# HanzhiC/TexPose

Hardware: AMD Instinct MI355X
Metric: rendered rays/sec (480x640x128 samples) + train iters/sec (higher is better)
Workload: dtype f32 carried as 2xf16 (f16x3 products, f32 accumulate); 1 GPU; Duck-like synthetic scene 480x640, 128 samples/ray, batch=1 image per GPU, forward render (render_by_slices mode='val', all pixels), per-sample outputs materialised; samples_per_ray=128, mlp_precision=f16x3, parallelism=images sharded across 1 GPU(s), no collective

## Files before the change

### texpose_amd/csrc/gen_wide_asm.py

```python
#!/usr/bin/env python3
import os
import sys

NCH = 115
EXPERIMENT = os.environ.get("TP_ASM_EXPERIMENT", "")
SPLIT = os.environ.get("TP_ASM_SPLIT", "mix")

VB = 160
def F_hi(slot): return VB + 8 * slot
def F_lo(slot): return VB + 8 * slot + 4
XB = [VB + 32, VB + 48]
T = VB + 64
VR = VB + 68
HACC = VB + 72
CLOBBER_V = list(range(XB[0], VR + 3))
BA, BB = 92, 94
CLOBBER_S = [BA, BA + 1, BB, BB + 1]
SET = {"P": 0, "Q": 128}


def vr(lo, n=4):
    return "v[%d:%d]" % (lo, lo + n - 1)


def ar(set_base, tile):
    lo = set_base + 16 * tile
    return "a[%d:%d]" % (lo, lo + 15)


def mfma(dst, a, b, c=None):
    return "v_mfma_f32_32x32x16_f16 %s, %s, %s, %s" % (dst, a, b, dst if c is None else c)


def conv(src_base, tile, g, bank):
    xh = XB[bank] + (g >> 2) * 4 + (g & 3)
    xl = XB[bank] + 8 + (g >> 2) * 4 + (g & 3)
    t0, t1, h0, h1 = T, T + 1, T + 2, T + 3
    a = src_base + 16 * tile + 2 * g
    head = ["v_accvgpr_read_b32 v%d, a%d" % (t0, a),
            "v_accvgpr_read_b32 v%d, a%d" % (t1, a + 1),
            "v_mul_f32 v%d, %%[kinv], v%d" % (t0, t0),
            "v_mul_f32 v%d, %%[kinv], v%d" % (t1, t1),
            "v_max_f32 v%d, 0, v%d" % (t0, t0),
            "v_max_f32 v%d, 0, v%d" % (t1, t1)]
    return head + split_ops(t0, t1, h0, h1, xh, xl) + ["v_pk_max_f16 %%[amax], %%[amax], v%d" % xh]


def split_ops(t0, t1, h0, h1, xh, xl):
    if SPLIT == "and":
        return ["v_and_b32 v%d, %%[mask], v%d" % (h0, t0),
                "v_and_b32 v%d, %%[mask], v%d" % (h1, t1),
                "v_sub_f32 v%d, v%d, v%d" % (t0, t0, h0),
                "v_sub_f32 v%d, v%d, v%d" % (t1, t1, h1),
                "v_cvt_pkrtz_f16_f32 v%d, v%d, v%d" % (xh, h0, h1),
                "v_cvt_pkrtz_f16_f32 v%d, v%d, v%d" % (xl, t0, t1)]
    return ["v_cvt_pkrtz_f16_f32 v%d, v%d, v%d" % (xh, t0, t1),
            "v_fma_mix_f32 v%d, -v%d, 1.0, v%d op_sel_hi:[1,0,0]" % (h0, xh, t0),
            "v_fma_mix_f32 v%d, -v%d, 1.0, v%d op_sel:[1,0,0] op_sel_hi:[1,0,0]" % (h1, xh, t1),
            "v_cvt_pkrtz_f16_f32 v%d, v%d, v%d" % (xl, h0, h1)]


MK = VB + 71
RB = 96


def rec_wr_off(r):
    return (r >> 2) * 4096 + (r & 3) * 128


def conv_rec(src_base, tile, g, bank, mask=True):
    c = conv(src_base, tile, g, bank)
    t0, t1 = T, T + 1
    r0, r1 = 2 * g, 2 * g + 1
    out = c[0:6]
    if EXPERIMENT != "recnolds":
        out += ["ds_write_b32 %%[recw], v%d offset:%d" % (t0, rec_wr_off(r0)),
                "ds_write_b32 %%[recw], v%d offset:%d" % (t1, rec_wr_off(r1))]
    else:
        out += ["s_nop 0", "s_nop 0"]
    if mask:
        out += ["v_cmp_lt_f32_e32 vcc, 0, v%d" % t0,
                "v_addc_co_u32_e32 v%d, vcc, v%d, v%d, vcc" % (MK, MK, MK),
                "v_cmp_lt_f32_e32 vcc, 0, v%d" % t1,
                "v_addc_co_u32_e32 v%d, vcc, v%d, v%d, vcc" % (MK, MK, MK)]
    out += c[6:]
    return out


def tile_regs(set_base, tile, k):
    lo = set_base + 16 * tile + 4 * k
    return "a[%d:%d]" % (lo, lo + 3)


def rec_reads(set_base, tile):
    if EXPERIMENT == "recnolds":
        return []
    return ["ds_read_b128 %s, %%[recr] offset:%d" % (tile_regs(set_base, tile, k), k * 4096) for k in range(4)]


def rec_store(set_base, tile, k):
    if EXPERIMENT in ("recnostore", "recnolds"):
        return "s_nop 0"
    policy = {"recplain": "", "recsc1": " sc1", "recsc01": " sc0 sc1"}.get(EXPERIMENT, " nt")
    return "global_store_dwordx4 %%[ro%d], %s, s[%d:%d] offset:%d%s" % (k & 1, tile_regs(set_base, tile, k), RB, RB + 1, (k >> 1) * 2048, policy)


def rec_advance():
    return ["s_add_u32 s%d, s%d, 0x1000" % (RB, RB), "s_addc_u32 s%d, s%d, 0" % (RB + 1, RB + 1)]


def rec_mask_store(w4):
    if EXPERIMENT in ("recnostore", "recnolds"):
        return []
    return ["v_bfrev_b32_e32 v%d, v%d" % (MK, MK),
            "global_store_dword %%[mkoff], v%d, %%[rbase] offset:%d" % (MK, w4 * 256)]


def split_even(instrs, n):
    k, out, pos = len(instrs), [], 0
    for i in range(n):
        take = (k - pos + (n - i) - 1) // (n - i)
        out.append(instrs[pos:pos + take])
        pos += take
    return out


def ring_prologue(e):
    e("s_waitcnt lgkmcnt(0)")
    e("s_nop 7")
    e("s_nop 7")
    e("s_lshl_b32 %[r0], %[buf], 15")
    for k, r in ((1, "r1"), (2, "r2")):
        e("s_add_i32 %%[t0], %%[buf], %d" % k)
        e("s_cmp_ge_i32 %[t0], 3")
        e("s_cselect_b32 %%[%s], 3, 0" % r)
        e("s_sub_i32 %%[t0], %%[t0], %%[%s]" % r)
        e("s_lshl_b32 %%[%s], %%[t0], 15" % r)
    for i, r in enumerate(("r0", "r1", "r2")):
        e("v_add_u32 v%d, %%[%s], %%[lane16]" % (VR + i, r))
        e("s_add_i32 %%[m%da], %%[ldswave], %%[%s]" % (i, r))
    e("s_add_i32 %[dch], %[chunk], 2")
    e("s_cmp_ge_i32 %[dch], %[nch]")
# ... 1 lines not shown
    e("s_sub_i32 %[dch], %[dch], %[t0]")


def dma_base():
    return ["s_lshl_b32 %[t0], %[dch], 15",
            "s_add_u32 s%d, %%[stream_lo], %%[t0]" % BA,
            "s_addc_u32 s%d, %%[stream_hi], 0" % (BA + 1),
            "s_add_u32 s%d, s%d, 0x1000" % (BB, BA),
            "s_addc_u32 s%d, s%d, 0" % (BB + 1, BA + 1)]


def dma_piece(e, k, dma_slot):
    if k == 0:
        e("s_mov_b32 m0, %%[m%da]" % dma_slot)
        e("s_nop 0")
    elif k == 4:
        e("s_add_i32 m0, %%[m%da], 0x1000" % dma_slot)
        e("s_nop 0")
    base = "s[%d:%d]" % ((BA, BA + 1) if k < 4 else (BB, BB + 1))
    if EXPERIMENT != "nodma":
        e("global_load_lds_dwordx4 %%[laneoff], %s offset:%d" % (base, (k & 3) * 1024))


def ring_epilogue(e, n_chunks):
    e("s_waitcnt lgkmcnt(0)")
    e("s_add_i32 %%[chunk], %%[chunk], %d" % n_chunks)
    e("s_cmp_ge_i32 %[chunk], %[nch]")
    e("s_cselect_b32 %[t0], %[nch], 0")
    e("s_sub_i32 %[chunk], %[chunk], %[t0]")
    e("s_add_i32 %%[buf], %%[buf], %d" % (n_chunks % 3))
    e("s_cmp_ge_i32 %[buf], 3")
    e("s_cselect_b32 %[t0], 3, 0")
    e("s_sub_i32 %[buf], %[buf], %[t0]")


def refill(e, slot, pair, npairs, cur, nxt):
    addr, off = (VR + cur, pair * 2048) if pair < npairs else (VR + nxt, (pair - npairs) * 2048)
    e("ds_read_b128 %s, v%d offset:%d" % (vr(F_hi(slot)), addr, off))
    e("ds_read_b128 %s, v%d offset:%d" % (vr(F_lo(slot)), addr, off + 1024))


def publish(e, young):
    e("s_waitcnt vmcnt(%d) lgkmcnt(0)" % (0 if EXPERIMENT == "nodma" else young))
    if EXPERIMENT != "nobarrier":
        e("s_barrier")


def chunk_groups(e, npairs, ts, mf, fill, free_after, pieces_per_group, tail=None, head=None, young_extra=0):
    ngroups = npairs // 2
    cur, nxt, dma = ts % 3, (ts + 1) % 3, (ts + 2) % 3
    pub_group = (npairs - 4) // 2
    for g in range(ngroups):
        q = 2 * g
        sa, sb = q % 4, (q + 1) % 4
        lines = mf(g)
        gaps = fill(g)
        e("s_waitcnt lgkmcnt(4)")
        for i in range(6):
            e(lines[i])
            if i == 0:
                for k in range(pieces_per_group):
                    dma_piece(e, g * pieces_per_group + k, dma)
                if head is not None:
                    for ins in head(g):
                        e(ins)
            if i < 5:
                for ins in gaps[i]:
                    e(ins)
            if i + 1 == free_after[0]:
                if g == pub_group:
                    publish(e, (g + 1) * pieces_per_group + (0 if EXPERIMENT in ("recnostore", "recnolds") else young_extra))
                refill(e, sa, q + 4, npairs, cur, nxt)
            if i + 1 == free_after[1]:
                refill(e, sb, q + 5, npairs, cur, nxt)
        if tail is not None:
            for ins in tail(g):
                e(ins)


def advance_dch():
    return ["s_add_i32 %[dch], %[dch], 1", "s_cmp_eq_u32 %[dch], %[nch]", "s_cselect_b32 %[dch], 0, %[dch]"]


def gen_wide(src, dst, rec=None):
    L = []
    e = L.append
    ring_prologue(e)
    cvf = (lambda *a: conv_rec(*a, mask=(rec == "mask"))) if rec else conv
    if rec:
        e("s_mov_b64 s[%d:%d], %%[rbase]" % (RB, RB + 1))
    for g in range(8):
        for ins in cvf(src, 0, g, 0):
            e(ins)
    if rec:
        for ins in rec_reads(src, 0):
            e(ins)
    for ins in dma_base():
        e(ins)
    for ts in range(8):
        bank = ts & 1

        def mf(g, bank=bank):
            s, t = g >> 2, (2 * g) & 7
            sa, sb = (2 * g) % 4, (2 * g + 1) % 4
            xh, xl = vr(XB[bank] + s * 4), vr(XB[bank] + 8 + s * 4)
            d0, d1 = ar(dst, t), ar(dst, t + 1)
            return [mfma(d0, vr(F_hi(sa)), xh), mfma(d1, vr(F_hi(sb)), xh), mfma(d0, vr(F_hi(sa)), xl),
                    mfma(d1, vr(F_hi(sb)), xl), mfma(d0, vr(F_lo(sa)), xh), mfma(d1, vr(F_lo(sb)), xh)]

        def fill(g, ts=ts, bank=bank):
            if rec:
                first, mid1, mid2, mid3, last = [], [], [], [], []
                if 1 <= g <= 4:
                    first = [rec_store(src, ts, g - 1)]
                if g == 5:
                    first = rec_advance()
                if g == 7 and ts < 7:
                    rd = rec_reads(src, ts + 1)
                    mid2, mid3 = mid2 + rd[0:2], mid3 + rd[2:4]
                    if rec == "mask" and not (ts & 1):
                        last = last + rec_mask_store(ts >> 1)
                if ts == 7:
                    return [first, mid1, mid2, mid3, last]
                cv = conv_rec(src, ts + 1, g, bank ^ 1, mask=(rec == "mask"))
                if rec == "mask":
                    return [first + cv[0:4], mid1 + cv[4:9], cv[9:14] + mid2, cv[14:18] + mid3, cv[18:19] + last]
                return [first + cv[0:4], mid1 + cv[4:8], cv[8:12] + mid2, cv[12:15] + mid3, last]
            if ts == 7:
                return [[], [], [], [], []]
            cv = conv(src, ts + 1, g, bank ^ 1)
            if EXPERIMENT == "noconv":
                return [[], [], [], [], []]
            return [[], cv[0:4], cv[4:8], cv[8:12], cv[12:13]]

        def tail(g, ts=ts):
            out = []
            if ts < 7:
                if 1 <= g <= 3:
                    out.append(advance_dch()[g - 1])
                if g == 7:
                    out += dma_base()
            return out

        def head(g, ts=ts):
            if g != (6 if rec else 0):
                return []
            return ["ds_read_b128 a[%d:%d], %%[nbias] offset:%d" % (src + 16 * ts + 4 * k, src + 16 * ts + 4 * k + 3, ts * 64 + k * 16)
                    for k in range(4)]

        extra = 0
        if rec:
            extra = 4 + (1 if (ts & 1) and rec == "mask" else 0)
        chunk_groups(e, 16, ts, mf, fill, (5, 6), 1, tail, head, young_extra=extra)
    ring_epilogue(e, 8)
    return L


def gen_extra(dst, ks):
    L = []
    e = L.append
    ring_prologue(e)
    for s in range(ks):
        e("ds_read_b128 %s, %%[stage] offset:%d" % (vr(XB[0] + s * 4), s * 8192))
        e("ds_read_b128 %s, %%[stage] offset:%d" % (vr(XB[0] + 8 + s * 4), s * 8192 + 4096))
    for ins in dma_base():
        e(ins)
    e("s_waitcnt lgkmcnt(0)")

    def mf(g):
        s, t = g >> 2, (2 * g) & 7
        sa, sb = (2 * g) % 4, (2 * g + 1) % 4
        xh, xl = vr(XB[0] + s * 4), vr(XB[0] + 8 + s * 4)
        d0, d1 = ar(dst, t), ar(dst, t + 1)
        return [mfma(d0, vr(F_hi(sa)), xh), mfma(d1, vr(F_hi(sb)), xh), mfma(d0, vr(F_hi(sa)), xl),
                mfma(d1, vr(F_hi(sb)), xl), mfma(d0, vr(F_lo(sa)), xh), mfma(d1, vr(F_lo(sb)), xh)]

    chunk_groups(e, 8 * ks, 0, mf, lambda g: [[], [], [], [], []], (5, 6), 2 // ks)
    ring_epilogue(e, 1)
    return L


def gen_head(src, rec=False):
    L = []
    e = L.append
    ring_prologue(e)
    if rec:
        e("s_mov_b64 s[%d:%d], %%[rbase]" % (RB, RB + 1))
    for g in range(8):
        for ins in (conv_rec(src, 0, g, 0) if rec else conv(src, 0, g, 0)):
            e(ins)
    def hold_reads(t):
        return rec_reads(src, t)

    if rec:
        for ins in hold_reads(0):
            e(ins)
    for ins in dma_base():
        e(ins)
    acc = vr(HACC, 16)

    def mf(g):
        bank = g & 1
        sa, sb = (2 * g) % 4, (2 * g + 1) % 4
        xh0, xh1 = vr(XB[bank]), vr(XB[bank] + 4)
        xl0, xl1 = vr(XB[bank] + 8), vr(XB[bank] + 12)
        first = mfma(acc, vr(F_hi(sa)), xh0, "0") if g == 0 else mfma(acc, vr(F_hi(sa)), xh0)
        return [first, mfma(acc, vr(F_hi(sa)), xl0), mfma(acc, vr(F_lo(sa)), xh0),
                mfma(acc, vr(F_hi(sb)), xh1), mfma(acc, vr(F_hi(sb)), xl1), mfma(acc, vr(F_lo(sb)), xh1)]

    def fill(g):
        cv = []
        if g < 7:
# ... 295 lines not shown
            vm += 1
        if q == n - 8:
            publish(e, vm)
            lg.drained()
        p = q + 8
        addr, off = (VR + cur, p * 1024) if p < n else (VR + nxt, (p - n) * 1024)
        lg.lds(e, "ds_read_b128 %s, v%d offset:%d" % (vr(F16(q % 8)), addr, off), slot=q % 8)
        for ins, is_lds in fill(q):
            if is_lds:
                lg.lds(e, ins)
            else:
                e(ins)
    for ins in (tail or []):
        e(ins)


def gen_wide16(src, dst):
    L = []
    e = L.append
    lg = Lgkm()
    ring_prologue(e)
    for ins in conv16_tile(src, 0, XB[0]):
        e(ins)
    for ins in dma_base():
        e(ins)
    for c in range(4):
        b = c & 1
        cv1 = split_even(conv16_tile(src, 2 * c + 1, XB[b] + 8), 15)
        cv2 = split_even(conv16_tile(src, 2 * c + 2, XB[b ^ 1]), 15) if c < 3 else [[] for _ in range(15)]

        def seed(tile, k):
            return ("ds_read_b128 a[%d:%d], %%[nbias] offset:%d" % (src + 16 * tile + 4 * k, src + 16 * tile + 4 * k + 3,
                                                                   tile * 64 + k * 16), True)

        def fill(q, c=c, cv1=cv1, cv2=cv2):
            out = []
            if 1 <= q <= 4:
                out.append(seed(2 * c, q - 1))
            if 17 <= q <= 20:
                out.append(seed(2 * c + 1, q - 17))
            if q < 15:
                out += [(i, False) for i in cv1[q]]
            elif 16 <= q < 31:
                out += [(i, False) for i in cv2[q - 16]]
            return out

        tail = advance_dch() + dma_base() if c < 3 else []
        chunk16(e, lg, c, 4, dst, lambda s, b=b: vr(XB[b] + 4 * s), fill, tail)
    ring_epilogue(e, 4)
    return L


def gen_extra16(dst, ks):
    L = []
    e = L.append
    lg = Lgkm()
    ring_prologue(e)
    for s in range(ks):
        e("ds_read_b128 %s, %%[stage] offset:%d" % (vr(XB[0] + 4 * s), s * 8192))
    for ins in dma_base():
        e(ins)
    e("s_waitcnt lgkmcnt(0)")
    chunk16(e, lg, 0, ks, dst, lambda s: vr(XB[0] + 4 * s), lambda q: [])
    ring_epilogue(e, 1)
    return L


def emit_macro(out, name, comment, lines):
    out.append("// " + comment)
    out.append("#define %s \\" % name)
    out.append(" \\\n".join('    "%s\\n"' % l for l in lines))
    out.append("")


def main():
    out = ["// GENERATED by gen_wide_asm.py -- do not edit.  See that file for the schedule.", "#pragma once",
           "#define TP_ASM_CLOBBERS " + ", ".join(['"v%d"' % v for v in CLOBBER_V] + ['"s%d"' % r for r in CLOBBER_S] + ['"a%d"' % a for a in range(256)]),
           "#define TP_ASM_ALL_AGPRS " + ", ".join('"a%d"' % a for a in range(256)),
           '#define TP_ASM_REC_CLOBBERS "v%d", "s%d", "s%d", "vcc"' % (MK, RB, RB + 1)]
    for s, d in (("Q", "P"), ("P", "Q")):
        emit_macro(out, "TP_ASM_WIDE_%s%s" % (s, d), "256 -> 256 layer: set %s -> set %s" % (s, d), gen_wide(SET[s], SET[d]))
        emit_macro(out, "TP_ASM_WIDE_%s%s_REC" % (s, d), "256 -> 256 layer: set %s -> set %s, recording set %s (values + ReLU sign words)" % (s, d, s),
                   gen_wide(SET[s], SET[d], rec="mask"))
    emit_macro(out, "TP_ASM_WIDE_QP_RECNM", "256 -> 256 layer: set Q -> set P, recording set Q (values only: the trunk feature)",
               gen_wide(SET["Q"], SET["P"], rec="nomask"))
    for d in ("P", "Q"):
        for ks in (1, 2):
            emit_macro(out, "TP_ASM_EXTRA%d_%s" % (ks, d), "%d extra k-step(s) into set %s" % (ks, d), gen_extra(SET[d], ks))
        emit_macro(out, "TP_ASM_HEAD_%s" % d, "narrow head over relu(set %s)" % d, gen_head(SET[d]))
        emit_macro(out, "TP_ASM_HEAD_%s_REC" % d, "narrow head over relu(set %s), recording set %s" % (d, d), gen_head(SET[d], rec=True))
        emit_macro(out, "TP_ASM_INIT_%s" % d, "seed set %s with the bias block" % d, gen_init(SET[d]))
        for t in range(8):
            emit_macro(out, "TP_ASM_READ_%s%d" % (d, t), "tile %d of set %s -> v[232:247]" % (t, d), gen_read_tile(SET[d], t))
    emit_macro(out, "TP_ASM_HEADV_P1", "fp32 VALU head, 1 row, over relu(set P)", gen_head_valu(SET["P"], HEADTAB_SIGMA))
    emit_macro(out, "TP_ASM_HEADV_P5", "fp32 VALU head, 5 rows, over relu(set P)", gen_head_valu(SET["P"], HEADTAB_TRANS))
    emit_macro(out, "TP_ASM_HEADV_Q3", "fp32 VALU head, 3 rows, over relu(set Q)", gen_head_valu(SET["Q"], HEADTAB_RGB))
    out.append("#define TP_HEADTAB_OFFSETS {%s}" % ", ".join(str(v) for v in HEADTAB_SIGMA + HEADTAB_TRANS + HEADTAB_RGB))
    emit_macro(out, "TP_ASM_STASH_Q", "set Q -> v[32:159]", gen_stash(SET["Q"]))
    emit_macro(out, "TP_ASM_RESTORE_P", "v[32:159] -> set P", gen_restore(SET["P"]))
    for s, d in (("Q", "P"), ("P", "Q")):
        emit_macro(out, "TP_ASM_WIDE16_%s%s" % (s, d), "f16: 256 -> 256 layer: set %s -> set %s" % (s, d), gen_wide16(SET[s], SET[d]))
    for d in ("P", "Q"):
        for ks in (1, 4):
            emit_macro(out, "TP_ASM_EXTRA16_%d_%s" % (ks, d), "f16: %d extra k-step(s) into set %s" % (ks, d), gen_extra16(SET[d], ks))
    emit_macro(out, "TP_ASM_DG_NARROW_P", "data gradient: set P = W3^T d (one k-step)", gen_dg_narrow(SET["P"]))
    emit_macro(out, "TP_ASM_DG_WIDE_PQ", "data gradient: set Q = W^T gated(set P), recording gated(set P)", gen_dg_wide(SET["P"], SET["Q"]))
    emit_macro(out, "TP_ASM_DG_WIDE_QP", "data gradient: set P = W^T gated(set Q), recording gated(set Q)", gen_dg_wide(SET["Q"], SET["P"]))
    emit_macro(out, "TP_ASM_DG_FINISH_P", "data gradient: record gated(set P)", gen_dg_finish(SET["P"]))
    sys.stdout.write("\n".join(out) + "\n")


if __name__ == "__main__":
    main()
```

### texpose_amd/csrc/mlp_fwd_f16x3.hip

```cpp
#include "mlp_mma.h"
#ifndef TP_WIDE_ASM_INC
#define TP_WIDE_ASM_INC "wide_asm.inc.h"
#endif
#include TP_WIDE_ASM_INC
#include <cstdlib>
#include <type_traits>

namespace {
using namespace tp_layout;
using namespace tp_mma;

using half8 = __attribute__((ext_vector_type(8))) _Float16;
using half2v = __attribute__((ext_vector_type(2))) __fp16;

constexpr int kBiasPad = (kBiasFloats + 63) / 64 * 64;
constexpr int kStageHalves = 5 * 2 * kThreads * 8;

constexpr int kBufs = 3;
constexpr int kSaveFloats = 8 * kThreads;
constexpr int kLdsBytes = kBufs * kChunkFloats * 4 + kBiasPad * 4 + kStageHalves * 2 + kSaveFloats * 4;
constexpr float kInvScale = 1.0f / (float)(1 << kF16WeightShift);

using u32x4 = __attribute__((ext_vector_type(4))) unsigned int;
__device__ __forceinline__ half8 pack8(const half2v (&p)[4]) {
// ... 222 lines not shown
struct AsmCtx { unsigned lane16, laneoff, ldswave, stream_lo, stream_hi, bias0, stage0; int nch; };
__device__ __forceinline__ AsmCtx asm_ctx_now(const float* packed, int nch = kNumChunks) {
  extern __shared__ __attribute__((aligned(16))) float lds_base[];
  int tid = threadIdx.x;
  asm volatile("" : "+v"(tid));
  const unsigned lane = (unsigned)tid & 63u, hh = ((unsigned)tid >> 5) & 1u;
  const unsigned wave = (unsigned)__builtin_amdgcn_readfirstlane(tid >> 6);
  AsmCtx c;
  const unsigned lds0 = (unsigned)(uintptr_t)AS3(lds_base);
  c.lane16 = lds0 + lane * 16u;
  c.laneoff = lane * 16u;
  c.ldswave = lds0 + wave * 8192u;
  const uint64_t sw = (uint64_t)(uintptr_t)(packed + wave * 2048);
  c.stream_lo = (unsigned)sw;
  c.stream_hi = (unsigned)(sw >> 32);
  const unsigned bias_lds = lds0 + (unsigned)(kBufs * kChunkFloats) * 4u;
  c.bias0 = bias_lds + hh * 512u;
  c.stage0 = bias_lds + (unsigned)kBiasPad * 4u + (unsigned)tid * 16u;
  c.nch = nch;
  return c;
}
#define TP_RING(f)                                                                                                     \
  "+{v[160:163]}"(f.h[0]), "+{v[164:167]}"(f.l[0]), "+{v[168:171]}"(f.h[1]), "+{v[172:175]}"(f.l[1]),                  \
      "+{v[176:179]}"(f.h[2]), "+{v[180:183]}"(f.l[2]), "+{v[184:187]}"(f.h[3]), "+{v[188:191]}"(f.l[3])
#define TP_RING_STATE                                                                                                  \
  [chunk] "+s"(chunk), [buf] "+s"(buf), [r0] "=&s"(r0), [r1] "=&s"(r1), [r2] "=&s"(r2), [m0a] "=&s"(m0a),              \
      [m1a] "=&s"(m1a), [m2a] "=&s"(m2a), [dch] "=&s"(dch), [t0] "=&s"(t0)
#define TP_RING_INPUTS(c)                                                                                              \
  [lane16] "v"(c.lane16), [laneoff] "v"(c.laneoff), [ldswave] "s"(__builtin_amdgcn_readfirstlane(c.ldswave)),         \
      [stream_lo] "s"(__builtin_amdgcn_readfirstlane(c.stream_lo)),                                                    \
      [stream_hi] "s"(__builtin_amdgcn_readfirstlane(c.stream_hi)), [nch] "s"(c.nch)
#define TP_ASM_HACC "v232", "v233", "v234", "v235", "v236", "v237", "v238", "v239", "v240", "v241", "v242", "v243", "v244", "v245", "v246", "v247"
#define TP_RING_LOCALS                                                                                                 \
  int chunk = __builtin_amdgcn_readfirstlane(p.chunk), buf = __builtin_amdgcn_readfirstlane(p.buf);                    \
  int r0, r1, r2, m0a, m1a, m2a, dch, t0
#define TP_RING_DONE                                                                                                   \
  p.chunk = chunk;                                                                                                     \
  p.buf = buf

#define TP_SF_OUT(F)                                                                                                   \
  "={v[32:47]}"(F[0]), "={v[48:63]}"(F[1]), "={v[64:79]}"(F[2]), "={v[80:95]}"(F[3]), "={v[96:111]}"(F[4]),            \
      "={v[112:127]}"(F[5]), "={v[128:143]}"(F[6]), "={v[144:159]}"(F[7])
#define TP_SF_IN(F)                                                                                                    \
  "{v[32:47]}"(F[0]), "{v[48:63]}"(F[1]), "{v[64:79]}"(F[2]), "{v[80:95]}"(F[3]), "{v[96:111]}"(F[4]),                 \
      "{v[112:127]}"(F[5]), "{v[128:143]}"(F[6]), "{v[144:159]}"(F[7])
__device__ __forceinline__ void asm_stash_q(f32x16 (&F)[8]) { asm volatile(TP_ASM_STASH_Q : TP_SF_OUT(F) : : TP_ASM_ALL_AGPRS); }
__device__ __forceinline__ void asm_restore_p(const f32x16 (&F)[8]) { asm volatile(TP_ASM_RESTORE_P : : TP_SF_IN(F) : TP_ASM_ALL_AGPRS); }
template <bool SET_P, int T>
__device__ __forceinline__ f32x16 asm_read_tile() {
  f32x16 v;
#define TP_RD(NAME) asm volatile(NAME : "={v[232:247]}"(v) : : TP_ASM_ALL_AGPRS)
  if constexpr (SET_P) {
    if constexpr (T == 0) TP_RD(TP_ASM_READ_P0); else if constexpr (T == 1) TP_RD(TP_ASM_READ_P1);
    else if constexpr (T == 2) TP_RD(TP_ASM_READ_P2); else if constexpr (T == 3) TP_RD(TP_ASM_READ_P3);
    else if constexpr (T == 4) TP_RD(TP_ASM_READ_P4); else if constexpr (T == 5) TP_RD(TP_ASM_READ_P5);
    else if constexpr (T == 6) TP_RD(TP_ASM_READ_P6); else TP_RD(TP_ASM_READ_P7);
  } else {
    if constexpr (T == 0) TP_RD(TP_ASM_READ_Q0); else if constexpr (T == 1) TP_RD(TP_ASM_READ_Q1);
    else if constexpr (T == 2) TP_RD(TP_ASM_READ_Q2); else if constexpr (T == 3) TP_RD(TP_ASM_READ_Q3);
    else if constexpr (T == 4) TP_RD(TP_ASM_READ_Q4); else if constexpr (T == 5) TP_RD(TP_ASM_READ_Q5);
    else if constexpr (T == 6) TP_RD(TP_ASM_READ_Q6); else TP_RD(TP_ASM_READ_Q7);
  }
#undef TP_RD
  return v;
}

template <bool SRC_Q>
__device__ __forceinline__ void asm_wide(Pipe& p, Frag& f, Guard& amax, const AsmCtx& c, int next_li) {
  TP_RING_LOCALS;
  const float kinv = kInvScale;
  const unsigned mask = 0xFFFFE000u;
  const unsigned nbias = c.bias0 + (unsigned)next_li * 1024u;
  if constexpr (SRC_Q)
    asm volatile(TP_ASM_WIDE_QP : TP_RING(f), TP_RING_STATE, [amax] "+v"(amax.m)
                 : TP_RING_INPUTS(c), [kinv] "s"(kinv), [mask] "s"(mask), [nbias] "v"(nbias)
                 : TP_ASM_CLOBBERS, TP_ASM_HACC, "memory", "scc");
  else
    asm volatile(TP_ASM_WIDE_PQ : TP_RING(f), TP_RING_STATE, [amax] "+v"(amax.m)
                 : TP_RING_INPUTS(c), [kinv] "s"(kinv), [mask] "s"(mask), [nbias] "v"(nbias)
                 : TP_ASM_CLOBBERS, TP_ASM_HACC, "memory", "scc");
  TP_RING_DONE;
}

template <bool SRC_Q>
__device__ __forceinline__ void asm_wide16(Pipe& p, Frag& f, Guard& amax, const AsmCtx& c, int next_li) {
  TP_RING_LOCALS;
  const unsigned nbias = c.bias0 + (unsigned)next_li * 1024u;
  if constexpr (SRC_Q)
    asm volatile(TP_ASM_WIDE16_QP : TP_RING(f), TP_RING_STATE, [amax] "+v"(amax.m)
                 : TP_RING_INPUTS(c), [nbias] "v"(nbias) : TP_ASM_CLOBBERS, "memory", "scc");
  else
    asm volatile(TP_ASM_WIDE16_PQ : TP_RING(f), TP_RING_STATE, [amax] "+v"(amax.m)
                 : TP_RING_INPUTS(c), [nbias] "v"(nbias) : TP_ASM_CLOBBERS, "memory", "scc");
  TP_RING_DONE;
}

struct RecCtx { unsigned recw, recr, ro0, ro1, mkoff; const float* rbase; };
__device__ __forceinline__ RecCtx rec_ctx_now(float* saved, int64_t tile, int slot) {
  extern __shared__ __attribute__((aligned(16))) float lds_base[];
  int tid = threadIdx.x;
  asm volatile("" : "+v"(tid));
  const unsigned lane = (unsigned)tid & 63u, j = (unsigned)tid & 31u, hh = ((unsigned)tid >> 5) & 1u;
  const unsigned wave = (unsigned)__builtin_amdgcn_readfirstlane(tid >> 6);
  const unsigned stg = (unsigned)(uintptr_t)AS3(lds_base) + (unsigned)(kBufs * kChunkFloats + kBiasPad) * 4u + wave * 1024u;
  RecCtx c;
  c.recw = stg + ((4u * hh) * 32u + j) * 4u;
  c.recr = stg + lane * 16u;
  c.ro0 = (unsigned)blk_off(0 + (int)(lane >> 3), (int)(lane & 7u) * 4) * 4u;
  c.ro1 = (unsigned)blk_off(8 + (int)(lane >> 3), (int)(lane & 7u) * 4) * 4u;
  static_assert(blk_off(16 + 3, 12) == blk_off(3, 12) + 512 && blk_off(24 + 6, 20) == blk_off(8 + 6, 20) + 512,
                "units 2 / 3 of a record tile sit 16 rows behind units 0 / 1 with the same swizzle");
  c.mkoff = (unsigned)((kMaskOff + ((slot > 0 ? slot : 1) - 1) * 256 - slot * kBlockFloats) * 4) + lane * 4u;
  const float* base = saved + (tile * 4 + (int64_t)wave) * (int64_t)kSavedGroupFloats + (int64_t)slot * kBlockFloats;
  const uint64_t b = (uint64_t)(uintptr_t)base;
  c.rbase = reinterpret_cast<const float*>((uint64_t)(unsigned)__builtin_amdgcn_readfirstlane((int)(unsigned)b) |
                                           ((uint64_t)(unsigned)__builtin_amdgcn_readfirstlane((int)(unsigned)(b >> 32)) << 32));
  return c;
}
#define TP_REC_INPUTS(r)                                                                                               \
  [recw] "v"(r.recw), [recr] "v"(r.recr), [ro0] "v"(r.ro0), [ro1] "v"(r.ro1), [mkoff] "v"(r.mkoff), [rbase] "s"(r.rbase)

template <class L>
constexpr int rec_kind_of() {
  if constexpr (std::is_same_v<L, int>) return 0;
  else return L::value == T0 ? 2 : (L::value == T1 || L::value == T2 || L::value == R1 || L::value == R2) ? 1 : 0;
}

template <bool SRC_Q, bool MASK>
__device__ __forceinline__ void asm_wide_rec(Pipe& p, Frag& f, Guard& amax, const AsmCtx& c, int next_li, const RecCtx& r) {
  TP_RING_LOCALS;
  const float kinv = kInvScale;
  const unsigned mask = 0xFFFFE000u;
  const unsigned nbias = c.bias0 + (unsigned)next_li * 1024u;
  static_assert(SRC_Q || MASK, "the mask-free variant exists for set Q only");
#define TP_WIDE_REC(TXT)                                                                                               \
  asm volatile(TXT : TP_RING(f), TP_RING_STATE, [amax] "+v"(amax.m)                                                    \
               : TP_RING_INPUTS(c), [kinv] "s"(kinv), [mask] "s"(mask), [nbias] "v"(nbias), TP_REC_INPUTS(r)           \
               : TP_ASM_CLOBBERS, TP_ASM_REC_CLOBBERS, "memory", "scc")
  if constexpr (SRC_Q && MASK) TP_WIDE_REC(TP_ASM_WIDE_QP_REC);
  else if constexpr (SRC_Q) TP_WIDE_REC(TP_ASM_WIDE_QP_RECNM);
  else TP_WIDE_REC(TP_ASM_WIDE_PQ_REC);
#undef TP_WIDE_REC
  TP_RING_DONE;
}

template <int KS, bool DST_P>
__device__ __forceinline__ void asm_extra(Pipe& p, Frag& f, const AsmCtx& c, int ks0) {
  TP_RING_LOCALS;
  const unsigned stage = c.stage0 + (unsigned)ks0 * 8192u;
#define TP_EXTRA(TXT)                                                                                                  \
  asm volatile(TXT : TP_RING(f), TP_RING_STATE : TP_RING_INPUTS(c), [stage] "v"(stage)                  \
               : TP_ASM_CLOBBERS, "memory", "scc")
  if constexpr (KS == 1 && DST_P) TP_EXTRA(TP_ASM_EXTRA1_P);
  else if constexpr (KS == 2 && DST_P) TP_EXTRA(TP_ASM_EXTRA2_P);
  else if constexpr (KS == 1) TP_EXTRA(TP_ASM_EXTRA1_Q);
  else TP_EXTRA(TP_ASM_EXTRA2_Q);
#undef TP_EXTRA
  TP_RING_DONE;
}

template <int KS, bool DST_P>
__device__ __forceinline__ void asm_extra16(Pipe& p, Frag& f, const AsmCtx& c, int ks0) {
  TP_RING_LOCALS;
  const unsigned stage = c.stage0 + (unsigned)ks0 * 8192u;
#define TP_EXTRA16(TXT)                                                                                                \
  asm volatile(TXT : TP_RING(f), TP_RING_STATE : TP_RING_INPUTS(c), [stage] "v"(stage) : TP_ASM_CLOBBERS, "memory", "scc")
// ... 35 lines not shown
                 "v244", "v245", "v246", "v247", "memory", "scc")
  if constexpr (SRC_P) TP_HEAD_REC(TP_ASM_HEAD_P_REC);
  else TP_HEAD_REC(TP_ASM_HEAD_Q_REC);
#undef TP_HEAD_REC
  TP_RING_DONE;
  return h;
}

struct Head5 { float r0, r1, r2, r3, r4; };
template <int WHICH>
__device__ __forceinline__ Head5 asm_head_valu(const Pipe& p, Frag& f, const AsmCtx& c) {
  int tid = threadIdx.x;
  asm volatile("" : "+v"(tid));
  const unsigned hw = c.stage0 - (unsigned)tid * 16u + (((unsigned)tid >> 5) & 1u) * 16u;
  const int buf = __builtin_amdgcn_readfirstlane(p.buf);
  int t0;
  Head5 h;
#define TP_HEADV(TXT)                                                                                                  \
  asm volatile(TXT : TP_RING(f), [t0] "=&s"(t0), "=&{v232}"(h.r0), "=&{v233}"(h.r1), "=&{v234}"(h.r2), "=&{v235}"(h.r3), \
                     "=&{v236}"(h.r4)                                                                                  \
               : [hw] "v"(hw), [lane16] "v"(c.lane16), [buf] "s"(buf)                                                  \
               : TP_ASM_CLOBBERS, "v231", "v237", "v238", "v239", "v240", "v241", "v242", "v243", "v244", "v245", "v246", "v247", \
                 "memory", "scc")
  if constexpr (WHICH == 0) TP_HEADV(TP_ASM_HEADV_P1);
  else if constexpr (WHICH == 1) TP_HEADV(TP_ASM_HEADV_P5);
  else TP_HEADV(TP_ASM_HEADV_Q3);
#undef TP_HEADV
  return h;
}

template <bool DST_P>
__device__ __forceinline__ void asm_init(const AsmCtx& c, int li) {
  const unsigned bias = c.bias0 + (unsigned)li * 1024u;
  if constexpr (DST_P) asm volatile(TP_ASM_INIT_P :: [bias] "v"(bias) : TP_ASM_CLOBBERS, "memory");
  else asm volatile(TP_ASM_INIT_Q :: [bias] "v"(bias) : TP_ASM_CLOBBERS, "memory");
}

struct Params {
  const float* packed;
  const float* center; const float* ray; const float* depth;
  const float* points; const float* ray_unit;
  const float* lat_trans; const float* lat_light;
  int B, R, N;
  int64_t n_samples, n_tiles;
  float* rgb; float* density; float* uncert; float* saved; float* workspace; int* status;
  const float* density_noise;
  unsigned int* act_max;
  const float* ray_bias;
};

__device__ __forceinline__ void stage(_Float16* st, int tid, int ks, int j, float v) {
  const _Float16 hi = (_Float16)v;
  st[((ks * 2 + 0) * kThreads + tid) * 8 + j] = hi;
  st[((ks * 2 + 1) * kThreads + tid) * 8 + j] = (_Float16)(v - (float)hi);
}

__device__ __forceinline__ void stage_slot(_Float16* st, int tid_lo, int slot, float v) {
  const int ks = slot >> 4, owner = tid_lo | ((slot & 8) << 2), jj = slot & 7;
  const _Float16 hi = (_Float16)v;
  st[((ks * 2 + 0) * kThreads + owner) * 8 + jj] = hi;
  st[((ks * 2 + 1) * kThreads + owner) * 8 + jj] = (_Float16)(v - (float)hi);
}

__device__ __forceinline__ float pick3(int c, float a0, float a1, float a2) {
  const uint32_t m0 = c == 0 ? 0xFFFFFFFFu : 0u, m1 = c == 1 ? 0xFFFFFFFFu : 0u, m2 = c == 2 ? 0xFFFFFFFFu : 0u;
  return __uint_as_float((__float_as_uint(a0) & m0) | (__float_as_uint(a1) & m1) | (__float_as_uint(a2) & m2));
}

#define TP_THREAD_IDS                                                                                                  \
  int tid = threadIdx.x;                                                                                               \
  asm volatile("" : "+v"(tid));                                                                                        \
  const int lane = tid & 63, j = tid & 31, hh = (tid >> 5) & 1;                                                        \
  const int wave = __builtin_amdgcn_readfirstlane(tid >> 6);                                                           \
  float* save = reinterpret_cast<float*>(st + kStageHalves) + tid;                                                     \
  (void)lane; (void)j; (void)hh; (void)wave; (void)save

template <bool SAVE, bool RB = false, bool F16 = false>
__global__ __launch_bounds__(kThreads, 1) void mlp_fwd_f16x3_kernel(Params P) {
  static_assert(!(SAVE && RB), "the ray-bias stream has no recording variant");
  static_assert(!(SAVE && F16), "the single-product arithmetic is inference only");
  constexpr int NCH = F16 ? (RB ? kNumChunks16RB : kNumChunks16) : (RB ? kNumChunksRB : kNumChunks);
  constexpr int BIAS_NCH = RB ? kNumChunksRB : kNumChunks;
  constexpr float kSetScale = F16 ? 1.0f : (float)(1 << kF16WeightShift);
#define TP_CTX asm_ctx_now(P.packed, NCH)
  extern __shared__ __attribute__((aligned(16))) float lds[];
  const int tid = threadIdx.x, lane = tid & 63, wave = tid >> 6;
  float* bias_lds = lds + kBufs * kChunkFloats;
  _Float16* st = reinterpret_cast<_Float16*>(bias_lds + kBiasPad);

  Pipe p;
  p.stream = P.packed; p.lds = lds; p.chunk = 0; p.buf = 0; p.wave = __builtin_amdgcn_readfirstlane(wave); p.lane = lane;
  for (int i = tid; i < kBiasFloats; i += kThreads)
    bias_lds[i] = P.packed[(size_t)BIAS_NCH * kChunkFloats + i] * (i < kHeadBiasOff ? kSetScale : 1.0f);
  if constexpr (RB) {
    constexpr int kHeadTabOff[kRbHeadRows] = TP_HEADTAB_OFFSETS;
    const float* tab = P.packed + kRbAuxOff + kRbAuxHeads;
    for (int i = tid; i < kRbHeadRows * 256; i += kThreads)
      *reinterpret_cast<float*>(reinterpret_cast<char*>(st) + kHeadTabOff[i >> 8] + (i & 255) * 4) =
          tab[i] * ((float)(1 << kF16WeightShift) / kSetScale);
  }
  dma_chunk(p, 0, 0);
  dma_chunk(p, 1, 1);
  __syncthreads();
  Frag frag;
  frag_prime(p, frag);
#ifdef TP_TRACE
  const long long tr_start = tick();
#endif
  asm_init<true>(TP_CTX, L0);

  for (int64_t tile = blockIdx.x; tile < P.n_tiles; tile += gridDim.x) {
    TR_BEGIN(pro);
    TP_THREAD_IDS;
    const int64_t s_raw = tile * 128 + wave * 32 + j;
    const bool live = s_raw < P.n_samples;
    const int64_t s = live ? s_raw : 0;
    const int64_t q = s / P.N;
    const int b = (int)(q / P.R);
    {
      float x0, x1, x2, vu0, vu1, vu2;
      if (P.center != nullptr) {
        const float z = P.depth[s];
        const float d0 = P.ray[3 * q + 0], d1 = P.ray[3 * q + 1], d2 = P.ray[3 * q + 2];
        x0 = tp::add_rn(P.center[3 * q + 0], tp::mul_rn(d0, z));
        x1 = tp::add_rn(P.center[3 * q + 1], tp::mul_rn(d1, z));
        x2 = tp::add_rn(P.center[3 * q + 2], tp::mul_rn(d2, z));
        float nrm = tp::add_rn(0.f, tp::mul_rn(d0, d0));
        nrm = tp::add_rn(nrm, tp::mul_rn(d1, d1));
        nrm = tp::add_rn(nrm, tp::mul_rn(d2, d2));
        const float den = fmaxf(sqrtf(nrm), 1e-12f);
        vu0 = tp::div_rn(d0, den); vu1 = tp::div_rn(d1, den); vu2 = tp::div_rn(d2, den);
      } else {
        x0 = P.points[3 * s + 0]; x1 = P.points[3 * s + 1]; x2 = P.points[3 * s + 2];
        vu0 = P.ray_unit[3 * s + 0]; vu1 = P.ray_unit[3 * s + 1]; vu2 = P.ray_unit[3 * s + 2];
      }
      save[0 * kThreads] = x0; save[1 * kThreads] = x1; save[2 * kThreads] = x2;
      if constexpr (!RB) {
        save[3 * kThreads] = vu0; save[4 * kThreads] = vu1; save[5 * kThreads] = vu2;
        save[6 * kThreads] = __int_as_float(b);
      } else {
        const int64_t qt = (tile * 128) / P.N;
        bias_lds[R0 * 256 + tid] = P.ray_bias[(size_t)P.B * 512 + (size_t)qt * 256 + tid] * (kSetScale * kInvScale);
        bias_lds[T0 * 256 + tid] = P.ray_bias[(size_t)(qt / P.R) * 512 + tid] * (kSetScale * kInvScale);
      }
    }
    asm_init<false>(TP_CTX, L1);
    TR_END(4, pro);
    f32x16 SF[8];
    Guard amax;
    float sig_s, rgb_s[3], ta0, ta1, ta2, ta3;
    const float* hbias = bias_lds + kHeadBiasOff;

    const auto head = [&](auto which_tag, auto after) {
      constexpr int which = decltype(which_tag)::value;
      TR_BEGIN(h);
      float a0, a1, a2, a3;
      if constexpr (SAVE && which != 0) {
        Head4 h4;
        if constexpr (which == 2) h4 = asm_head_rec<false>(p, frag, amax, TP_CTX, rec_ctx_now(P.saved, tile, SV_R2));
        else h4 = asm_head_rec<true>(p, frag, amax, TP_CTX, rec_ctx_now(P.saved, tile, SV_T2));
        a0 = h4.a0; a1 = h4.a1; a2 = h4.a2; a3 = h4.a3;
        TR_END(7, h);
      } else if constexpr (RB) {
        const Head5 h5 = asm_head_valu<which>(p, frag, TP_CTX);
        TR_END(7, h);
        TP_THREAD_IDS;
        a0 = (which == 1 && hh) ? h5.r4 : h5.r0; a1 = h5.r1; a2 = h5.r2; a3 = h5.r3;
      } else {
        f32x16 a;
        if constexpr (which == 2) a = asm_head<false>(p, frag, amax, TP_CTX, 1.0f / kSetScale);
        else a = asm_head<true>(p, frag, amax, TP_CTX, 1.0f / kSetScale);
        TR_END(7, h);
        a0 = a[0]; a1 = a[1]; a2 = a[2]; a3 = a[3];
      }
      after();
      if (which == 0) {
        float dn = 0.0f;
        if (P.density_noise != nullptr) {
          TP_THREAD_IDS;
          int64_t sn = tile * 128 + wave * 32 + j;
          if (sn >= P.n_samples) sn = P.n_samples - 1;
          dn = P.density_noise[sn];
        }
        sig_s = softplus(fmaf(a0, kInvScale, hbias[0]) + dn);
      } else if (which == 1) {
        ta0 = a0; ta1 = a1; ta2 = a2; ta3 = a3;
      } else {
        rgb_s[0] = sigmoid(fmaf(a0, kInvScale, hbias[6])); rgb_s[1] = sigmoid(fmaf(a1, kInvScale, hbias[7]));
        rgb_s[2] = sigmoid(fmaf(a2, kInvScale, hbias[8]));
      }
    };

    const auto layer = [&](auto even_tag, auto li_arg) {
      constexpr bool EVEN = decltype(even_tag)::value;
      const int li = li_arg;
      constexpr int REC = SAVE ? rec_kind_of<decltype(li_arg)>() : 0;
      if (!EVEN && li == L7) head(std::integral_constant<int, 0>{}, [] {});
      if (!EVEN && li == R0)
        head(std::integral_constant<int, 1>{}, [&] {
          TR_BEGIN(rl);
          asm_restore_p(SF);
          TR_END(10, rl);
        });

      if (li != L0) {
        TR_BEGIN(w);
        const int next_li = li + 1 == kNumWide ? 0 : li + 1;
        if constexpr (REC == 2) asm_wide_rec<true, false>(p, frag, amax, TP_CTX, next_li, rec_ctx_now(P.saved, tile, SV_FEAT));
        else if constexpr (REC == 1) asm_wide_rec<EVEN, true>(p, frag, amax, TP_CTX, next_li, rec_ctx_now(P.saved, tile, li - 1 - L7));
        else if constexpr (F16) asm_wide16<EVEN>(p, frag, amax, TP_CTX, next_li);
        else asm_wide<EVEN>(p, frag, amax, TP_CTX, next_li);
        TR_END(3, w);
      }

      if (EVEN && (li == L0 || li == L4)) {
        TR_BEGIN(pe);
        if (li == L0) {
          TP_THREAD_IDS;
          const float x0 = save[0 * kThreads], x1 = save[1 * kThreads], x2 = save[2 * kThreads];
#ifdef TP_PE_PER_OCTAVE
#pragma unroll 5
          for (int i = 0; i < 15; ++i) {
            const int pi_ = hh * 15 + i, c = (pi_ * 205) >> 11, l = pi_ - c * 10;
            const float xc = pick3(c, x0, x1, x2);
            float sv, cv;
            tp::sincos_both(tp::mul_rn(xc, ldexpf(3.14159274101257324f, l)), sv, cv);
            stage_slot(st, tid & ~32, 20 * c + l, sv);
            stage_slot(st, tid & ~32, 20 * c + 10 + l, cv);
          }
#else
          const int ca = 2 * hh;
          tp::SinCos64 ea = tp::sincos_f64(tp::mul_rn(hh ? x2 : x0, 3.14159274101257324f));
          tp::SinCos64 eb = tp::sincos_f64(tp::mul_rn(x1, 3.14159274101257324f));
#pragma unroll
          for (int l = 0; l < 10; ++l) {
            stage_slot(st, tid & ~32, 20 * ca + l, (float)ea.s);
            stage_slot(st, tid & ~32, 20 * ca + 10 + l, (float)ea.c);
            stage_slot(st, tid & ~32, 20 + 10 * hh + l, (float)(hh ? eb.c : eb.s));
            if (l < 9) { tp::sincos_double(ea); tp::sincos_double(eb); }
          }
#endif
          if (hh) {
            stage(st, tid, 3, 4, x0); stage(st, tid, 3, 5, x1); stage(st, tid, 3, 6, x2); stage(st, tid, 3, 7, 0.0f);
          }
        }
        TR_END(5, pe);
        TR_BEGIN(w);
        if constexpr (F16) {
          asm_extra16<4, true>(p, frag, TP_CTX, 0);
        } else {
          asm_extra<2, true>(p, frag, TP_CTX, 0);
          asm_extra<2, true>(p, frag, TP_CTX, 2);
        }
        TR_END(3, w);
      } else if (RB && EVEN && li == T0) {
      } else if (RB && !EVEN && li == R0) {
        TR_BEGIN(r0s);
        TP_THREAD_IDS;
        if (hh == 0) {
          save[0 * kThreads] = sigmoid(fmaf(ta0, kInvScale, hbias[1]));
          save[1 * kThreads] = sigmoid(fmaf(ta1, kInvScale, hbias[2]));
          save[2 * kThreads] = sigmoid(fmaf(ta2, kInvScale, hbias[3]));
          save[3 * kThreads] = softplus(fmaf(ta3, kInvScale, hbias[4]));
        } else {
          save[0 * kThreads] = softplus(fmaf(ta0, kInvScale, hbias[5]));
        }
        TR_END(6, r0s);
        TR_BEGIN(w);
        if constexpr (F16) asm_extra16<1, false>(p, frag, TP_CTX, 3);
        else asm_extra<1, false>(p, frag, TP_CTX, 3);
        TR_END(3, w);
      } else if (EVEN && li == T0) {
        TR_BEGIN(t0s);
        TP_THREAD_IDS;
        const int bt = __float_as_int(save[6 * kThreads]);
#pragma unroll
        for (int jj = 0; jj < 8; ++jj) stage(st, tid, 0, jj, P.lat_trans[bt * 16 + 8 * hh + jj]);
        TR_END(13, t0s);
        TR_BEGIN(w);
        if constexpr (F16) asm_extra16<1, true>(p, frag, TP_CTX, 0);
        else asm_extra<1, true>(p, frag, TP_CTX, 0);
        TR_END(3, w);
      } else if (!EVEN && li == R0) {
        TR_BEGIN(r0s);
        TP_THREAD_IDS;
        float* sx = SAVE ? P.saved + (tile * 4 + wave) * (int64_t)kSavedGroupFloats + SV_EX * kBlockFloats : nullptr;
        const float x0 = save[0 * kThreads], x1 = save[1 * kThreads], x2 = save[2 * kThreads];
        const float vu0 = save[3 * kThreads], vu1 = save[4 * kThreads], vu2 = save[5 * kThreads];
        const int br = __float_as_int(save[6 * kThreads]);
#ifdef TP_PE_PER_OCTAVE
#pragma unroll 3
        for (int i = 0; i < 6; ++i) {
          const int pi_ = hh * 6 + i, c = pi_ >> 2, l = pi_ & 3;
          const float vc = pick3(c, vu0, vu1, vu2);
          float sv, cv;
// ... 4 lines not shown
        }
#else
        {
          const int ca = 2 * hh;
          tp::SinCos64 ea = tp::sincos_f64(tp::mul_rn(hh ? vu2 : vu0, 3.14159274101257324f));
          tp::SinCos64 eb = tp::sincos_f64(tp::mul_rn(vu1, 3.14159274101257324f));
#pragma unroll
          for (int l = 0; l < 4; ++l) {
            const float sa = (float)ea.s, cav = (float)ea.c, vb = (float)(hh ? eb.c : eb.s);
            const int s0 = 3 + 8 * ca + l, s1 = 3 + 8 + 4 * hh + l;
            stage_slot(st, tid & ~32, s0, sa);
            stage_slot(st, tid & ~32, s0 + 4, cav);
            stage_slot(st, tid & ~32, s1, vb);
            if (SAVE && live) { sx[blk_off(s0, j)] = sa; sx[blk_off(s0 + 4, j)] = cav; sx[blk_off(s1, j)] = vb; }
            if (l < 3) { tp::sincos_double(ea); tp::sincos_double(eb); }
          }
        }
#endif
        if (hh == 0) {
          stage(st, tid, 0, 0, vu0); stage(st, tid, 0, 1, vu1); stage(st, tid, 0, 2, vu2);
          if (SAVE && live) { sx[blk_off(0, j)] = vu0; sx[blk_off(1, j)] = vu1; sx[blk_off(2, j)] = vu2; }
        } else {
          stage(st, tid, 1, 3, x0); stage(st, tid, 1, 4, x1); stage(st, tid, 1, 5, x2);
          stage(st, tid, 1, 6, P.lat_light[br * 48 + 0]); stage(st, tid, 1, 7, P.lat_light[br * 48 + 1]);
          if (SAVE && live) { sx[blk_off(27, j)] = x0; sx[blk_off(28, j)] = x1; sx[blk_off(29, j)] = x2; }
        }
#pragma unroll
        for (int ks = 2; ks < 5; ++ks) {
          float lv[8];
#pragma unroll
          for (int jj = 0; jj < 8; ++jj) {
            const int slot = 16 * ks + 8 * hh + jj;
            lv[jj] = slot < 78 ? P.lat_light[br * 48 + slot - 30] : 0.0f;
          }
          half8 hi8, lo8;
#pragma unroll
          for (int jj = 0; jj < 8; ++jj) {
            hi8[jj] = (_Float16)lv[jj];
            lo8[jj] = (_Float16)(lv[jj] - (float)hi8[jj]);
          }
          *reinterpret_cast<half8*>(st + ((ks * 2 + 0) * kThreads + tid) * 8) = hi8;
          *reinterpret_cast<half8*>(st + ((ks * 2 + 1) * kThreads + tid) * 8) = lo8;
        }
        if (hh == 0) {
          save[0 * kThreads] = sigmoid(fmaf(ta0, kInvScale, hbias[1]));
          save[1 * kThreads] = sigmoid(fmaf(ta1, kInvScale, hbias[2]));
          save[2 * kThreads] = sigmoid(fmaf(ta2, kInvScale, hbias[3]));
          save[3 * kThreads] = softplus(fmaf(ta3, kInvScale, hbias[4]));
        } else {
          save[0 * kThreads] = softplus(fmaf(ta0, kInvScale, hbias[5]));
        }
        TR_END(6, r0s);
        TR_BEGIN(w);
        if constexpr (F16) {
          asm_extra16<4, false>(p, frag, TP_CTX, 0);
          asm_extra16<1, false>(p, frag, TP_CTX, 4);
        } else {
          asm_extra<2, false>(p, frag, TP_CTX, 0);
          asm_extra<2, false>(p, frag, TP_CTX, 2);
          asm_extra<1, false>(p, frag, TP_CTX, 4);
        }
        TR_END(3, w);
      }

      if (!EVEN && li == L7) {
        TR_BEGIN(vc);
        asm_stash_q(SF);
        TR_END(9, vc);
      }
    };

    if constexpr (SAVE) {
#pragma nounroll
      for (int pr = 0; pr < 4; ++pr) {
        layer(std::true_type{}, 2 * pr);
        layer(std::false_type{}, 2 * pr + 1);
      }
      layer(std::true_type{}, std::integral_constant<int, T0>{});
      layer(std::false_type{}, std::integral_constant<int, T1>{});
      layer(std::true_type{}, std::integral_constant<int, T2>{});
      layer(std::false_type{}, std::integral_constant<int, R0>{});
      layer(std::true_type{}, std::integral_constant<int, R1>{});
      layer(std::false_type{}, std::integral_constant<int, R2>{});
    } else {
#pragma nounroll
      for (int pr = 0; pr < kNumWide / 2; ++pr) {
        layer(std::true_type{}, 2 * pr);
        layer(std::false_type{}, 2 * pr + 1);
      }
    }
    head(std::integral_constant<int, 2>{}, [] {});

    TR_BEGIN(o);
    {
      TP_THREAD_IDS;
      int64_t so = tile * 128 + wave * 32 + j;
      asm volatile("" : "+v"(so));
      if (so < P.n_samples) {
        if (hh == 0) {
          float* o = P.rgb + so * 6;
#pragma unroll
          for (int c = 0; c < 3; ++c) {
            __builtin_nontemporal_store(rgb_s[c], o + 2 * c);
            __builtin_nontemporal_store(save[c * kThreads], o + 2 * c + 1);
          }
          __builtin_nontemporal_store(sig_s, P.density + so * 2);
          __builtin_nontemporal_store(save[3 * kThreads], P.density + so * 2 + 1);
        } else {
          __builtin_nontemporal_store(save[0 * kThreads], P.uncert + so);
        }
      }
    }
    const float tile_max = fmaxf((float)amax.m[0], (float)amax.m[1]);
    if (P.status != nullptr && !(tile_max < 6.0e4f)) atomicOr(P.status, 1);
    if (P.act_max != nullptr) {
      int lid;
      asm volatile("v_mbcnt_lo_u32_b32 %0, -1, 0\n\tv_mbcnt_hi_u32_b32 %0, -1, %0" : "=v"(lid));
      float wmax = tile_max;
#pragma unroll
      for (int off = 32; off >= 1; off >>= 1)
        wmax = fmaxf(wmax, __int_as_float(__builtin_amdgcn_ds_bpermute((lid ^ off) << 2, __float_as_int(wmax))));
      if (lid == 0 && wmax == wmax) atomicMax(P.act_max, __float_as_uint(wmax));
    }
    TR_END(11, o);
  }
#ifdef TP_TRACE
  if (lane == 0 && blockIdx.x == 100 && wave == 1 && P.n_tiles > 1000) {
    const long long tot = tick() - tr_start;
    printf("trace total %lld | dma %lld vm %lld bar %lld wide %lld | pro %lld pe %lld r0 %lld heads %lld | init %lld park %lld reload %lld out %lld | gen0 %lld t0stage %lld\n",
           tot, p.tr[0], p.tr[1], p.tr[2], p.tr[3], p.tr[4], p.tr[5], p.tr[6], p.tr[7], p.tr[8], p.tr[9], p.tr[10], p.tr[11], p.tr[12], p.tr[13]);
  }
#endif
}
#undef TP_CTX

__global__ __launch_bounds__(256) void rb_image_bias_kernel(const float* __restrict__ packed, const float* __restrict__ lat_trans,
                                                            const float* __restrict__ lat_light, float* __restrict__ out) {
  const int b = blockIdx.x, e = threadIdx.x;
  const int h = e >> 7, t = (e >> 4) & 7, r = e & 15, f = feat_of(t, r, h);
  const float* bias = packed + (size_t)kNumChunksRB * kChunkFloats;
  const float* aux = packed + kRbAuxOff;
  float at = bias[bias_index(T0, h, t, r)];
#pragma unroll
  for (int c = 0; c < 16; ++c) at = fmaf(aux[kRbAuxTrans + c * 256 + f], lat_trans[b * 16 + c], at);
  float al = bias[bias_index(R0, h, t, r)];
#pragma unroll 8
  for (int c = 0; c < 48; ++c) al = fmaf(aux[kRbAuxLight + c * 256 + f], lat_light[b * 48 + c], al);
  out[(size_t)b * 512 + e] = at * (float)(1 << kF16WeightShift);
  out[(size_t)b * 512 + 256 + e] = al;
}

constexpr int kRbRays = 32;
__global__ __launch_bounds__(256) void rb_ray_bias_kernel(const float* __restrict__ packed, const float* __restrict__ ray, int R,
                                                          int64_t n_rays, const float* __restrict__ img, float* __restrict__ out) {
  __shared__ float enc[kRbRays][28];
  const int e = threadIdx.x;
  const int64_t q0 = (int64_t)blockIdx.x * kRbRays;
  if (e < kRbRays * 3) {
    const int i = e / 3, c = e - 3 * i;
    const int64_t q = q0 + i < n_rays ? q0 + i : n_rays - 1;
    const float d0 = ray[3 * q + 0], d1 = ray[3 * q + 1], d2 = ray[3 * q + 2];
    float nrm = tp::add_rn(0.f, tp::mul_rn(d0, d0));
    nrm = tp::add_rn(nrm, tp::mul_rn(d1, d1));
    nrm = tp::add_rn(nrm, tp::mul_rn(d2, d2));
    const float den = fmaxf(sqrtf(nrm), 1e-12f);
    const float vu = tp::div_rn(c == 0 ? d0 : (c == 1 ? d1 : d2), den);
// ... 475 lines not shown
```

Measured before the change: 2.054 million rays/s.

## Fold density head row into L7 wide layer's conversion pass

Adds a generated asm variant of the P->Q wide layer that, while converting relu(set P) tiles to f16 pairs, also multiplies the fp32 values by the sigma head row read from LDS and accumulates into two VGPRs, then reduces across lanes with permlane32 swap. In the ray-bias, non-f16 forward path the L7 layer now uses it, so the separate sigma head pass over set P is skipped. The layer loop is split so L7 is a compile-time layer. This costs extra LDS reads, VALU FMAs and waitcnts inside the tightly scheduled MFMA loop, and it uses more VGPRs.

```diff
diff --git a/texpose_amd/csrc/gen_wide_asm.py b/texpose_amd/csrc/gen_wide_asm.py
--- a/texpose_amd/csrc/gen_wide_asm.py
+++ b/texpose_amd/csrc/gen_wide_asm.py
@@ -58,6 +58,20 @@
             "v_fma_mix_f32 v%d, -v%d, 1.0, v%d op_sel_hi:[1,0,0]" % (h0, xh, t0),
             "v_fma_mix_f32 v%d, -v%d, 1.0, v%d op_sel:[1,0,0] op_sel_hi:[1,0,0]" % (h1, xh, t1),
             "v_cvt_pkrtz_f16_f32 v%d, v%d, v%d" % (xl, h0, h1)]
+
+
+SGW = VB + 72
+
+
+def sig_reads(tile, k):
+    return "ds_read_b128 %s, %%[hw] offset:%d" % (vr(SGW + 4 * k), HEADTAB_SIGMA[0] + (4 * tile + k) * 32)
+
+
+def conv_sig(src_base, tile, g, bank, first=False):
+    c = conv(src_base, tile, g, bank)
+    op = "v_mul_f32 %%[sg%d], v%d, v%d" if first else "v_fmac_f32 %%[sg%d], v%d, v%d"
+    fma = [op % (0, T, SGW + 2 * g), op % (1, T + 1, SGW + 2 * g + 1)]
+    return (c[0:6] + fma + c[6:]) if SPLIT == "and" else (c + fma)
 
 
 MK = VB + 71
@@ -225,14 +239,31 @@
     return ["s_add_i32 %[dch], %[dch], 1", "s_cmp_eq_u32 %[dch], %[nch]", "s_cselect_b32 %[dch], 0, %[dch]"]
 
 
-def gen_wide(src, dst, rec=None):
+def wait_before_sig(lst, n):
+    i = next(k for k, ins in enumerate(lst) if "%[sg" in ins)
+    lst.insert(i, "s_waitcnt lgkmcnt(%d)" % n)
+
+
+def gen_wide(src, dst, rec=None, sig=False):
+    assert not (rec and sig)
     L = []
     e = L.append
     ring_prologue(e)
+    if sig:
+        L[3:3] = [sig_reads(0, k) for k in range(4)]
     cvf = (lambda *a: conv_rec(*a, mask=(rec == "mask"))) if rec else conv
     if rec:
         e("s_mov_b64 s[%d:%d], %%[rbase]" % (RB, RB + 1))
     for g in range(8):
+        if sig:
+            cv = conv_sig(src, 0, g, 0, first=(g == 0))
+            if not (g & 1):
+                wait_before_sig(cv, 3)
+            else:
+                cv.append(sig_reads(1, g >> 1))
+            for ins in cv:
+                e(ins)
+            continue
         for ins in cvf(src, 0, g, 0):
             e(ins)
     if rec:
@@ -271,6 +302,14 @@
                 return [first + cv[0:4], mid1 + cv[4:8], cv[8:12] + mid2, cv[12:15] + mid3, last]
             if ts == 7:
                 return [[], [], [], [], []]
+            if sig:
+                cv = conv_sig(src, ts + 1, g, bank ^ 1)
+                gaps = [[], cv[0:4], cv[4:8], cv[8:12], cv[12:]] if SPLIT == "and" else [[], cv[0:4], cv[4:8], cv[8:11], cv[11:]]
+                if ts == 0 and g == 0:
+                    wait_before_sig(gaps[1] if SPLIT == "and" else gaps[4], 7)
+                if (g & 1) and ts < 6:
+                    gaps[4].append(sig_reads(ts + 2, g >> 1))
+                return gaps
             cv = conv(src, ts + 1, g, bank ^ 1)
             if EXPERIMENT == "noconv":
                 return [[], [], [], [], []]
@@ -732,6 +771,8 @@
         emit_macro(out, "TP_ASM_WIDE_%s%s" % (s, d), "256 -> 256 layer: set %s -> set %s" % (s, d), gen_wide(SET[s], SET[d]))
         emit_macro(out, "TP_ASM_WIDE_%s%s_REC" % (s, d), "256 -> 256 layer: set %s -> set %s, recording set %s (values + ReLU sign words)" % (s, d, s),
                    gen_wide(SET[s], SET[d], rec="mask"))
+    emit_macro(out, "TP_ASM_WIDE_PQ_SIG", "256 -> 256 layer: set P -> set Q, with the density row over relu(set P) (ray-bias form, L7)",
+               gen_wide(SET["P"], SET["Q"], sig=True))
     emit_macro(out, "TP_ASM_WIDE_QP_RECNM", "256 -> 256 layer: set Q -> set P, recording set Q (values only: the trunk feature)",
                gen_wide(SET["Q"], SET["P"], rec="nomask"))
     for d in ("P", "Q"):
diff --git a/texpose_amd/csrc/mlp_fwd_f16x3.hip b/texpose_amd/csrc/mlp_fwd_f16x3.hip
--- a/texpose_amd/csrc/mlp_fwd_f16x3.hip
+++ b/texpose_amd/csrc/mlp_fwd_f16x3.hip
@@ -328,6 +328,24 @@
   TP_RING_DONE;
 }
 
+__device__ __forceinline__ float asm_wide_sig(Pipe& p, Frag& f, Guard& amax, const AsmCtx& c, int next_li) {
+  TP_RING_LOCALS;
+  const float kinv = kInvScale;
+  const unsigned mask = 0xFFFFE000u;
+  const unsigned nbias = c.bias0 + (unsigned)next_li * 1024u;
+  int tid = threadIdx.x;
+  asm volatile("" : "+v"(tid));
+  const unsigned hw = c.stage0 - (unsigned)tid * 16u + (((unsigned)tid >> 5) & 1u) * 16u;
+  float sg0, sg1;
+  asm volatile(TP_ASM_WIDE_PQ_SIG : TP_RING(f), TP_RING_STATE, [amax] "+v"(amax.m), [sg0] "=&v"(sg0), [sg1] "=&v"(sg1)
+               : TP_RING_INPUTS(c), [kinv] "s"(kinv), [mask] "s"(mask), [nbias] "v"(nbias), [hw] "v"(hw)
+               : TP_ASM_CLOBBERS, TP_ASM_HACC, "memory", "scc");
+  TP_RING_DONE;
+  float x = sg0 + sg1, y = x;
+  asm volatile("s_nop 1\n\tv_permlane32_swap_b32 %0, %1\n\ts_nop 1" : "+v"(x), "+v"(y));
+  return x + y;
+}
+
 template <bool SRC_Q>
 __device__ __forceinline__ void asm_wide16(Pipe& p, Frag& f, Guard& amax, const AsmCtx& c, int next_li) {
   TP_RING_LOCALS;
@@ -529,6 +547,11 @@
   constexpr int NCH = F16 ? (RB ? kNumChunks16RB : kNumChunks16) : (RB ? kNumChunksRB : kNumChunks);
   constexpr int BIAS_NCH = RB ? kNumChunksRB : kNumChunks;
   constexpr float kSetScale = F16 ? 1.0f : (float)(1 << kF16WeightShift);
+#ifdef TP_HEADS_PARENT
+  constexpr bool SIGFOLD = false;
+#else
+  constexpr bool SIGFOLD = RB && !F16;
+#endif
 #define TP_CTX asm_ctx_now(P.packed, NCH)
   extern __shared__ __attribute__((aligned(16))) float lds[];
   const int tid = threadIdx.x, lane = tid & 63, wave = tid >> 6;
@@ -642,7 +665,8 @@
       constexpr bool EVEN = decltype(even_tag)::value;
       const int li = li_arg;
       constexpr int REC = SAVE ? rec_kind_of<decltype(li_arg)>() : 0;
-      if (!EVEN && li == L7) head(std::integral_constant<int, 0>{}, [] {});
+      constexpr bool SIG_L7 = SIGFOLD && !EVEN && !std::is_same_v<decltype(li_arg), int>;
+      if (!SIG_L7 && !EVEN && li == L7) head(std::integral_constant<int, 0>{}, [] {});
       if (!EVEN && li == R0)
         head(std::integral_constant<int, 1>{}, [&] {
           TR_BEGIN(rl);
@@ -656,8 +680,21 @@
         if constexpr (REC == 2) asm_wide_rec<true, false>(p, frag, amax, TP_CTX, next_li, rec_ctx_now(P.saved, tile, SV_FEAT));
         else if constexpr (REC == 1) asm_wide_rec<EVEN, true>(p, frag, amax, TP_CTX, next_li, rec_ctx_now(P.saved, tile, li - 1 - L7));
         else if constexpr (F16) asm_wide16<EVEN>(p, frag, amax, TP_CTX, next_li);
-        else asm_wide<EVEN>(p, frag, amax, TP_CTX, next_li);
-        TR_END(3, w);
+        else if constexpr (SIG_L7) {
+          const float a0 = asm_wide_sig(p, frag, amax, TP_CTX, next_li);
+          TR_END(3, w);
+          TR_BEGIN(h);
+          float dn = 0.0f;
+          if (P.density_noise != nullptr) {
+            TP_THREAD_IDS;
+            int64_t sn = tile * 128 + wave * 32 + j;
+            if (sn >= P.n_samples) sn = P.n_samples - 1;
+            dn = P.density_noise[sn];
+          }
+          sig_s = softplus((a0 + hbias[0]) + dn);
+          TR_END(7, h);
+        } else asm_wide<EVEN>(p, frag, amax, TP_CTX, next_li);
+        if constexpr (!SIG_L7) TR_END(3, w);
       }
 
       if (EVEN && (li == L0 || li == L4)) {
@@ -828,6 +865,20 @@
       layer(std::false_type{}, std::integral_constant<int, R0>{});
       layer(std::true_type{}, std::integral_constant<int, R1>{});
       layer(std::false_type{}, std::integral_constant<int, R2>{});
+    } else if constexpr (SIGFOLD) {
+      static_assert(L7 == 7 && (kNumWide & 1) == 0, "L0 .. L6 | L7 | T0 .. R2");
+#pragma nounroll
+      for (int pr = 0; pr < 3; ++pr) {
+        layer(std::true_type{}, 2 * pr);
+        layer(std::false_type{}, 2 * pr + 1);
+      }
+      layer(std::true_type{}, 6);
+      layer(std::false_type{}, std::integral_constant<int, L7>{});
+#pragma nounroll
+      for (int pr = 4; pr < kNumWide / 2; ++pr) {
+        layer(std::true_type{}, 2 * pr);
+        layer(std::false_type{}, 2 * pr + 1);
+      }
     } else {
 #pragma nounroll
       for (int pr = 0; pr < kNumWide / 2; ++pr) {
```

New measurement: 2.055 million rays/s (median of 2 runs). No clear change (+0.0%).
